# ddrainer/FloodPlanet_Code

Hardware: AMD Instinct MI355X
Metric: training tiles/sec (256x256x8ch UNet) (higher is better)
Workload: dtype bf16; 1 GPU; UNet depth-4 (17.27M params), 8-band 256x256 tiles, batch 16/GPU, fwd+CE(ignore_index=0)+bwd+Adam, train-mode BN; global_batch=16, parallelism=dp1

## Files before the change

floodplanet_code_amd/_lib.py:

```python
from __future__ import annotations

import ctypes as C
import os
from typing import Optional

_HERE = os.path.dirname(os.path.abspath(__file__))
LIB_PATH = os.environ.get("FU_LIB_PATH") or os.path.join(_HERE, "libfloodunet.so")

FU_OK, FU_ERR_INVALID, FU_ERR_HIP, FU_ERR_STATE, FU_ERR_UNSUPPORTED = 0, 1, 2, 3, 4
FU_F32, FU_BF16, FU_F16 = 0, 1, 2
PRECISIONS = {"fp32": FU_F32, "f32": FU_F32, "float32": FU_F32, "bf16": FU_BF16, "bfloat16": FU_BF16,
              "fp16": FU_F16, "f16": FU_F16, "float16": FU_F16, "half": FU_F16}


class FuConfig(C.Structure):
    _fields_ = [
        ("struct_size", C.c_int32),
        ("n_channels", C.c_int32),
        ("n_classes", C.c_int32),
        ("base_channels", C.c_int32),
        ("bilinear", C.c_int32),
        ("max_batch", C.c_int32),
        ("height", C.c_int32),
        ("width", C.c_int32),
# ... 126 lines not shown
    "fu_profile_enable": (_i, [_p, _i]),
    "fu_test_force_general_conv": (None, [_i]),
    "fu_test_force_lockstep_wgrad": (None, [_i]),
    "fu_test_conv_tile_mode": (None, [_i]),
    "fu_test_bnb_separate": (None, [_i]),
    "fu_test_head_store_g": (None, [_i]),
    "fu_test_force_full_taps": (None, [_i]),
    "fu_test_perturb_bnb_sums": (None, [_f]),
    "fu_test_get_buffer": (_i, [_p, _i, _i, C.POINTER(_p), C.POINTER(_i64)]),
    "fu_set_side_stream": (_i, [_p, _i]),
    "fu_backward_join": (_i, [_p, _p]),
    "fu_backward_fence": (_i, [_p, _p, _p]),
    "fu_dp_unique_id": (_i, [_p]),
    "fu_dp_init": (_i, [_p, _p, _i, _i]),
    "fu_dp_broadcast_state": (_i, [_p, _p]),
    "fu_allreduce_begin": (_i, [_p, _i64, _i64, _p]),
    "fu_allreduce_wait": (_i, [_p, _p]),
    "fu_dp_destroy": (_i, [_p]),
    "fu_set_exact_sync": (_i, [_p, SYNC_HOOK, _p, _i, _p, _i64]),
    "fu_exact_sync_bytes": (_i64, [_p]),
    "fu_profile_read": (_i, [_p, _i, C.POINTER(_i64), C.POINTER(C.c_double), C.POINTER(C.c_double),
                             C.POINTER(C.c_char_p)]),
    "fu_elem_size": (_i, [_i]),
    "fu_op_nchw_to_nhwc": (_i, [_i, _p, _p, _i, _i, _i, _i, _i, _p]),
    "fu_op_nhwc_to_nchw": (_i, [_i, _p, _p, _i, _i, _i, _i, _i, _p]),
    "fu_op_conv3x3_fwd": (_i, [_i, _p, _i, _p, _p, _p, _i, _p, _p, _p, _i, _i, _i, _i, _p, _p, _p]),
    "fu_op_conv3x3_dgrad": (_i, [_i, _p, _i, _p, _p, _i, _p, _i, _i, _i, _i, _p]),
    "fu_op_conv3x3_wgrad": (_i, [_i, _p, _i, _p, _p, _p, _i, _p, _i, _p, _i, _i, _i, _p]),
    "fu_op_conv3x3_dgrad_bnsums": (_i, [_i, _p, _i, _p, _p, _i, _p, _p, _p, _p, _p, _p, _p, _i, _i, _i, _p]),
    "fu_op_head_bwd": (_i, [_i, _p, _p, _p, _p, _p, _i, _i, _i64, _p, _p, _p, _p, _p, _p, _p, _p]),
    "fu_op_bn_bwd": (_i, [_i, _p, _p, _i, _i, _i, _i, _p, _p, _p, _p, _p, _p, _p, _p]),
    "fu_op_maxpool2": (_i, [_i, _p, _p, _p, _p, _i, _i, _i, _i, _p]),
    "fu_op_upsample2": (_i, [_i, _p, _p, _p, _p, _i, _i, _i, _i, _i, _i, _p]),
}

_lib: Optional[C.CDLL] = None


def load() -> C.CDLL:
    global _lib
    if _lib is not None:
        return _lib
    if not os.path.exists(LIB_PATH):
        raise RuntimeError(
            f"{LIB_PATH} not found: the HIP extension has not been built. Run "
            "`python -c 'import __graft_entry__ as g; g.build()'` (or `make -C floodplanet_code_amd/csrc`). "
            "There is no CPU / PyTorch fallback for this path.")
    import torch
    lib = C.CDLL(LIB_PATH)
    for name, (res, args) in SIGNATURES.items():
        fn = getattr(lib, name)
        fn.restype = res
        fn.argtypes = args
    _lib = lib
    return lib


def check(status: int) -> None:
    if status != FU_OK:
        msg = load().fu_last_error()
        raise FloodUNetError(status, msg.decode("utf-8", "replace") if msg else "")


def ptr(t) -> Optional[int]:
    return None if t is None else t.data_ptr()
```

floodplanet_code_amd/csrc/fu_api.hip:

```cpp
#include "../../include/floodunet.h"
#include "fu_common.h"
#include <stdlib.h>

#include <math.h>
#include <string.h>

#include <string>
#include <vector>

using namespace fu;

namespace fu {

int conv3x3_num_stat_tiles(Prec p, int B, int H, int W) {
  return p == PREC_F32 ? conv3x3_num_stat_tiles_f32(B, H, W)
                       : (p == PREC_BF16 ? conv3x3_num_stat_tiles_bf16(B, H, W) : conv3x3_num_stat_tiles_f16(B, H, W));
}
int launch_conv3x3(Prec p, const ConvIn& in, const void* wpk, const float* bias, void* dst0, int D0, void* dst1,
                   int D1, float* stats, int* n_stat_tiles, int B, int H, int W, hipStream_t s) {
  if (p == PREC_F32)
    return launch_conv3x3_f32(in, (const float*)wpk, bias, (float*)dst0, D0, (float*)dst1, D1, stats, n_stat_tiles, B,
                              H, W, s);
  if (p == PREC_BF16)
    return launch_conv3x3_bf16(in, (const bf16_t*)wpk, bias, (bf16_t*)dst0, D0, (bf16_t*)dst1, D1, stats, n_stat_tiles,
// ... 162 lines not shown
  const int c = blockIdx.x * blockDim.x + threadIdx.x;
  if (c >= C) return;
  const float invstd = (float)(1.0 / sqrt((double)rv[c] + (double)eps));
  const float sc = gamma[c] * invstd;
  scale[c] = sc;
  fbias[c] = fmaf(sc, bias[c], beta[c] - rm[c] * sc);
  a[c] = 1.f;
  b[c] = 0.f;
}

struct ParamInfo {
  std::string name;
  int ndim;
  int64_t shape[4];
  int64_t off, numel;
};
struct BnInfo {
  std::string name;
  int C;
  int64_t off;
};

struct Conv {
  int cin_real = 0, cin_pad = 0, cout = 0, level = 0;
  int p_w = -1, p_b = -1, p_g = -1, p_beta = -1, bn = -1;
  void* wf = nullptr;
  void* wd = nullptr;
  float *mean = nullptr, *invstd = nullptr, *a = nullptr, *b = nullptr, *coef = nullptr;
  float *fold_scale = nullptr, *fold_bias = nullptr;
  void* y = nullptr;
  void* gy = nullptr;
  const void* pool_g = nullptr;
  int bnb_tiles = 0;
  HeadGrad head;
};

enum BlockKind { BK_INC = 0, BK_DOWN = 1, BK_UP = 2 };

struct Block {
  Conv c[2];
  int kind = BK_INC, level = 0;
  int enc = 0;
  int role = 0;
  int skip = -1;
  void* pooled = nullptr;
  void* g_pooled = nullptr;
  void* up = nullptr;
  void* g_up = nullptr;
  UpTables upt;
  int ct_w = -1, ct_b = -1, ct_cin = 0, ct_cout = 0;
  void* u = nullptr;
  void* g_u = nullptr;
  float* ct_w3 = nullptr;
  float* ct_dw3 = nullptr;
  float* ct_b4 = nullptr;
  void* ct_wf = nullptr;
  void* ct_wd = nullptr;
  int first_param = 0, num_params = 0;
};

struct Fuse {
  int p_w = -1, p_b = -1, C = 0;
  void* cat = nullptr;
  void* gcat = nullptr;
  void* y = nullptr;
  void* gy = nullptr;
// ... 42 lines not shown
struct Dp;
struct fu_ctx {
  fu_config cfg;
  Prec prec;
  size_t esize;
  int Hs[5], Ws[5], ch[5];
  int nE = 1;
  bool fusion = false;
  int nb = 9;
  int enc_ch[FU_MAX_ENCODERS] = {0}, enc_coff[FU_MAX_ENCODERS] = {0}, cin_pad0[FU_MAX_ENCODERS] = {0};
  void* xin[FU_MAX_ENCODERS] = {nullptr};
  std::vector<ParamInfo> params;
  std::vector<BnInfo> bns;
  int64_t total_params = 0, total_bn = 0;
  std::vector<Block> blk;
  Fuse fuse[5];
  int p_outw = -1, p_outb = -1;
  float* P = nullptr;
  float* G = nullptr;
  float* RM = nullptr;
  float* RV = nullptr;
  int64_t* NBT = nullptr;
  bool packed_dirty = true;
  bool packed_eval = false;
  Arena arena;
  std::vector<void*> extra_allocs;
  float* logits = nullptr;
  float* dlogits = nullptr;
  float* dlogits_eff = nullptr;
  float* up_scale = nullptr;
  bool have_up_scale = false;
  float* stats = nullptr;
  float* bnb_part = nullptr;
  int64_t bnb_cap = 0;
  float* db_part = nullptr;
  float* db_part2 = nullptr;
  hipStream_t side = nullptr;
  hipStream_t side_lo = nullptr;
  hipStream_t side_def = nullptr;
  hipEvent_t ev_gy = nullptr, ev_wg[2] = {nullptr, nullptr}, ev_blk = nullptr;
  hipEvent_t ev_fence[2] = {nullptr, nullptr};
  int wg_parity = 0;
  int side_mode = 1;
  bool wg_pending[2] = {false, false};
  double* dscratch = nullptr;
  fu::SyncDesc sync;
  float* slab = nullptr;
  float* ce_part = nullptr;
  float* hb_part = nullptr;
  float* loss_dev = nullptr;
  float* ce_wsum = nullptr;
  float* loss_scale = nullptr;
  int* guard = nullptr;
  unsigned long long* conf_tmp = nullptr;
  int64_t* n_valid = nullptr;
  DeviceTable stitch_table, scene_table, train_table;
  float* adam_m = nullptr;
  float* adam_v = nullptr;
  Profiler prof;
  struct Dp* dp = nullptr;
  std::vector<PackTable> pack_tabs;
  int last_batch = 0;
  int view_n = 0;
  int view_batch = 0;
  unsigned view_codes = 0;
  bool fwd_training = false;
// ... 474 lines not shown
                         f.n_classes, B, f.height, f.width, c->logits, logits_out, s));
  c->last_batch = B;
  c->view_n = n_views;
  c->view_batch = n_views > 0 ? B / n_views : 0;
  c->view_codes = view_codes;
  c->fwd_training = training;
  c->have_loss = false;
  c->have_up_scale = false;
  return 0;
}

static int g_bnb_separate = 0;
static int g_head_store_g = 0;
static float g_test_perturb_bnb = 1.f;
__global__ void k_scale_floats(float* x, int64_t n, float f) {
  for (int64_t i = (int64_t)blockIdx.x * blockDim.x + threadIdx.x; i < n; i += (int64_t)gridDim.x * blockDim.x) x[i] *= f;
}
int perturb_bnb(float* part, int tiles, int C, hipStream_t s) {
  if (g_test_perturb_bnb == 1.f || tiles <= 0) return 0;
  hipLaunchKernelGGL(k_scale_floats, dim3(256), dim3(256), 0, s, part, (int64_t)tiles * C * 2, g_test_perturb_bnb);
  return hipGetLastError() == hipSuccess ? 0 : FU_ERR_HIP;
}

int backward_conv(fu_ctx* c, int i, int j, int B, hipStream_t s) {
  Block& K = c->blk[i];
  Conv& v = K.c[j];
  const int H = c->Hs[v.level], W = c->Ws[v.level];
  const int64_t npix = (int64_t)B * H * W;
  int ndb = 0;
  const bool side = c->side != nullptr && c->side_mode != 0;
  const int par = c->wg_parity;
  float* dbp = (side && par) ? c->db_part2 : c->db_part;
  if (side && c->wg_pending[par]) FU_HIP_CHECK(hipStreamWaitEvent(s, c->ev_wg[par], 0));
  FU_TRY(launch_bn_bwd(c->prec, v.gy, v.y, v.cout, npix, v.a, v.b, v.mean, v.invstd, P(c, v.p_g), G(c, v.p_g),
                       G(c, v.p_beta), c->bnb_part, v.coef, dbp, &ndb, c->dscratch, s, v.pool_g, B, H, W, v.bnb_tiles,
                       v.head.dl ? &v.head : nullptr));
  v.pool_g = nullptr;
  v.bnb_tiles = 0;
  v.head = HeadGrad{};
  ConvIn in = conv_input(c, i, j);
  const double fl = 2.0 * 9 * v.cin_real * v.cout * (double)B * H * W;
  hipStream_t ws = s;
  if (side) {
    FU_HIP_CHECK(hipEventRecord(c->ev_gy, s));
    FU_HIP_CHECK(hipStreamWaitEvent(c->side, c->ev_gy, 0));
    ws = c->side;
  }
  in.opt.prof = prof_arm(c, FU_K_WGRAD, fl);
  FU_TRY(launch_conv3x3_wgrad(c->prec, in, v.gy, v.cout, c->slab, G(c, v.p_w), v.cin_real, dbp, ndb,
                              G(c, v.p_b), B, H, W, ws));
  if (side) {
    FU_HIP_CHECK(hipEventRecord(c->ev_wg[par], c->side));
    c->wg_pending[par] = true;
    c->wg_parity ^= 1;
  }
  ConvIn din{v.gy, v.cout, nullptr, nullptr, nullptr, 0};
  if (!(K.role == 0 && j == 0)) din.opt.prof = prof_arm(c, FU_K_CONV3X3, fl);
  if (j == 1) {
    Conv& v0 = K.c[0];
    const bool separate = g_bnb_separate != 0;
    int tiles = 0;
    BnbFuse f;
    if (c->prec != PREC_F32 && !c->sync.hook && !separate) {
      f.y = v0.y; f.a = v0.a; f.b = v0.b; f.mean = v0.mean; f.invstd = v0.invstd;
      f.part = c->bnb_part; f.max_elems = c->bnb_cap; f.tiles_out = &tiles;
      din.opt.bnb = &f;
    }
    FU_TRY(launch_conv3x3(c->prec, din, v.wd, nullptr, v0.gy, v0.cout, nullptr, 0, nullptr, nullptr, B, H, W, s));
    v0.bnb_tiles = tiles;
    FU_TRY(perturb_bnb(c->bnb_part, tiles, v0.cout, s));
  } else if (K.kind == BK_DOWN) {
    FU_TRY(launch_conv3x3(c->prec, din, v.wd, nullptr, K.g_pooled, v.cin_real, nullptr, 0, nullptr, nullptr, B, H, W,
                          s));
    Conv& pv = c->blk[i - 1].c[1];
    pv.pool_g = K.g_pooled;
  } else if (K.kind == BK_UP) {
    const Feat sk = level_feat(c, K.skip);
    const Feat pv = low_feat(c, i);
    FU_TRY(launch_conv3x3(c->prec, din, v.wd, nullptr, sk.gy, sk.C, K.g_up, v.cin_real - sk.C, nullptr, nullptr,
                          B, H, W, s));
    const int h = c->Hs[K.level + 1], w = c->Ws[K.level + 1];
    if (c->cfg.bilinear) {
      FU_TRY(launch_upsample2_bwd(c->prec, K.g_up, pv.gy, B, h, w, pv.C, H, W, K.upt, s));
    } else {
      FU_TRY(launch_space_to_depth(c->prec, K.g_up, K.g_u, B, h, w, K.ct_cout, H, W, s));
      int ndbp = 0;
      FU_TRY(launch_channel_partial_sums(c->prec, K.g_u, K.ct_cout, (int64_t)B * h * w * 4, c->db_part, &ndbp, s));
      FU_TRY(launch_colsum_partials(c->db_part, ndbp, K.ct_cout, G(c, K.ct_b), s));
      ConvIn lin{pv.y, pv.C, pv.a, pv.b, nullptr, 0, true};
      FU_TRY(launch_conv3x3_wgrad(c->prec, lin, K.g_u, 4 * K.ct_cout, c->slab, K.ct_dw3, K.ct_cin, nullptr, 0, nullptr, B, h,
                                  w, s));
      FU_TRY(launch_convT_grad_from_w3(K.ct_dw3, K.ct_cin, K.ct_cout, G(c, K.ct_w), s));
      ConvIn gin{K.g_u, 4 * K.ct_cout, nullptr, nullptr, nullptr, 0, true};
      FU_TRY(launch_conv3x3(c->prec, gin, K.ct_wd, nullptr, pv.gy, K.ct_cin, nullptr, 0, nullptr, nullptr, B, h, w, s));
    }
  }
  return 0;
}

int num_backward_blocks(const fu_ctx* c) { return 5 + (c->fusion ? 1 : 0) + 5 * c->nE; }
int backward_block_index(const fu_ctx* c, int block) {
  if (block <= 4) return c->nb - block;
  const int k = block - 5 - (c->fusion ? 1 : 0);
  return 5 * c->nE - 1 - k;
}

int backward_block_impl(fu_ctx* c, int block, const float* dlogits_ext, hipStream_t s, bool join) {
  const fu_config& f = c->cfg;
  const int B = c->last_batch;
  if (block == 0) {
    if (dlogits_ext) {
      FU_TRY(launch_dlogits_from_nchw(dlogits_ext, c->dlogits, f.n_classes, B, f.height, f.width, s));
      c->have_up_scale = false;
    } else {
      FU_REQUIRE(c->have_loss, "fu_backward: no dlogits given and no fu_loss_* call since the last forward");
    }
    const float* dl = c->dlogits;
    if (c->prec == PREC_F16 || c->have_up_scale) {
      FU_TRY(launch_loss_grad_eff(c->dlogits, c->dlogits_eff, (int64_t)B * f.height * f.width * f.n_classes,
                                  c->have_up_scale ? c->up_scale : nullptr, c->ce_part,
                                  c->prec == PREC_F16 ? c->loss_scale : nullptr, s,
                                  c->prec == PREC_F16 ? c->guard : nullptr));
      dl = c->dlogits_eff;
    }
    Conv& last = c->blk[c->nb - 1].c[1];
    BnbFuse fz;
    int tiles = 0;
    const bool want = c->prec != PREC_F32 && !c->sync.hook && !g_bnb_separate;
    if (want) {
      fz.y = last.y; fz.a = last.a; fz.b = last.b; fz.mean = last.mean; fz.invstd = last.invstd;
      fz.part = c->bnb_part; fz.max_elems = c->bnb_cap; fz.tiles_out = &tiles;
      fz.skip_g = last.cout % 8 == 0 && 2048 % last.cout == 0 && !g_head_store_g;
    }
    FU_TRY(launch_head_bwd(c->prec, dl, last.y, last.a, last.b, P(c, c->p_outw), f.base_channels, f.n_classes,
                           (int64_t)B * f.height * f.width, last.gy, c->hb_part, G(c, c->p_outw), G(c, c->p_outb), s,
                           want ? &fz : nullptr));
    last.bnb_tiles = tiles;
    FU_REQUIRE(!(want && fz.skip_g) || tiles > 0, "head backward: the fused BatchNorm sums were refused (partials %lld floats)",
               (long long)c->bnb_cap);
    last.head = HeadGrad{};
    if (want && fz.skip_g) { last.head.dl = dl; last.head.w = P(c, c->p_outw); last.head.ncls = f.n_classes; }
    FU_TRY(perturb_bnb(c->bnb_part, tiles, last.cout, s));
    return 0;
// ... 934 lines not shown
  FU_TRY(launch_head_bwd(p, dlogits_nhwc, y, bn_a, bn_b, w, C, ncls, npix, g, (float*)part.p, dw, db, s,
                         want ? &f : nullptr));
  if (want) {
    if (tiles <= 0) {
      set_error("fu_op_head_bwd: the head-backward kernel does not emit the sums in this precision");
      return FU_ERR_UNSUPPORTED;
    }
    FU_TRY(perturb_bnb((float*)bpart.p, tiles, C, s));
    FU_TRY(collapse_partials((const float*)bpart.p, tiles, C, sum_gm, sum_gmx, s));
  }
  FU_HIP_CHECK(hipStreamSynchronize(s));
  return FU_OK;
}

int fu_op_bn_bwd(int precision, void* g, const void* y, int C, int B, int H, int W, const float* bn_a,
                 const float* bn_b, const float* mean, const float* invstd, const void* g_pool, float* dgamma,
                 float* dbeta, fu_stream stream) {
  Prec p; FU_TRY(prec_of(precision, &p));
  FU_REQUIRE(g && y && bn_a && bn_b && mean && invstd && dgamma && dbeta, "fu_op_bn_bwd: null argument");
  hipStream_t s = (hipStream_t)stream;
  const int64_t npix = (int64_t)B * H * W;
  TmpBuf part, coef, dbp, scr;
  FU_TRY(part.get((size_t)bn_bwd_partial_elems(C, npix) * sizeof(float)));
  FU_TRY(coef.get((size_t)C * 2 * sizeof(float)));
  FU_TRY(dbp.get((size_t)bn_bwd_partial_elems(C, npix) * sizeof(float)));
  FU_TRY(scr.get((size_t)reduce_scratch_elems(std::max(C, 64)) * sizeof(double)));
  int ndb = 0;
  FU_TRY(launch_bn_bwd(p, g, y, C, npix, bn_a, bn_b, mean, invstd, nullptr, dgamma, dbeta, (float*)part.p,
                       (float*)coef.p, (float*)dbp.p, &ndb, (double*)scr.p, s, g_pool, B, H, W, 0));
  FU_HIP_CHECK(hipStreamSynchronize(s));
  return FU_OK;
}

int fu_test_get_buffer(fu_ctx* c, int block, int which, void** ptr, int64_t* elems) {
  FU_REQUIRE(c && ptr && elems, "fu_test_get_buffer: null argument");
  FU_REQUIRE(block >= 0 && block < c->nb, "fu_test_get_buffer: block %d outside 0..%d", block, c->nb - 1);
  const Block& K = c->blk[block];
  const int B = c->cfg.max_batch;
  auto act = [&](int level, int C) { return (int64_t)B * c->Hs[level] * c->Ws[level] * C; };
  switch (which) {
    case 0: *ptr = K.c[0].y; *elems = act(K.c[0].level, K.c[0].cout); break;
    case 1: *ptr = K.c[0].gy; *elems = act(K.c[0].level, K.c[0].cout); break;
    case 2: *ptr = K.c[1].y; *elems = act(K.c[1].level, K.c[1].cout); break;
    case 3: *ptr = K.c[1].gy; *elems = act(K.c[1].level, K.c[1].cout); break;
    case 4: *ptr = K.g_pooled; *elems = K.kind == BK_DOWN ? act(K.level, K.c[0].cin_real) : 0; break;
    case 5: *ptr = K.g_up; *elems = K.kind == BK_UP ? act(K.level, K.c[0].cin_real - c->ch[K.skip]) : 0; break;
    default: set_error("fu_test_get_buffer: which must be 0..5"); return FU_ERR_INVALID;
  }
  return FU_OK;
}

}

extern "C" void fu_test_bnb_separate(int on) { g_bnb_separate = on ? 1 : 0; }
extern "C" void fu_test_head_store_g(int on) { g_head_store_g = on ? 1 : 0; }
extern "C" void fu_test_perturb_bnb_sums(float factor) { g_test_perturb_bnb = factor; }
```

floodplanet_code_amd/csrc/fu_common.h:

```cpp
#pragma once
#include <hip/hip_runtime.h>
#include <stdint.h>
#include <stdio.h>
#include <string>

struct fu_stitch_entry;
struct fu_scene_crop;
struct fu_scene_train_entry;

namespace fu {

typedef unsigned short bf16_t;
struct f16_t { unsigned short v; };

enum Prec { PREC_F32 = 0, PREC_BF16 = 1, PREC_F16 = 2 };

template <typename F> auto dispatch_prec(Prec p, F&& f) {
  if (p == PREC_F32) return f(float{});
  if (p == PREC_BF16) return f(bf16_t{});
  return f(f16_t{});
}

void set_error(const char* fmt, ...);
const char* get_error();
// ... 300 lines not shown
                        int src_channels = 0, int src_channel_offset = 0);
int launch_nhwc_to_nchw(Prec p, const void* src, float* dst, int B, int C, int H, int W, int c_pad, hipStream_t s);
struct SrcList { const float* p[8]; int c[8]; int coff[9]; int n; };
int launch_gather_nchw_to_nhwc(Prec p, const SrcList& S, void* dst, int B, int C, int H, int W, int c_pad, int ch_off,
                               hipStream_t s);
int launch_gather_views_nchw_to_nhwc(Prec p, const SrcList& S, void* dst, int B, int n_views, unsigned codes, int C, int H,
                                     int W, int c_pad, int ch_off, hipStream_t s);

int launch_bn_finalize(const float* partials, int nTiles, int C, int64_t count, const float* conv_bias,
                       const float* gamma, const float* beta, float eps, float momentum, float* mean, float* invstd,
                       float* a, float* b, float* running_mean, float* running_var, int64_t* nbt, double* dscratch,
                       hipStream_t s);
static inline int64_t reduce_scratch_elems(int C) { return (int64_t)32 * C * 2; }
int64_t bn_bwd_partial_elems(int C, int64_t npix);
int launch_bn_bwd(Prec p, void* g, const void* y, int C, int64_t npix, const float* a, const float* b,
                  const float* mean, const float* invstd, const float* gamma, float* dgamma, float* dbeta,
                  float* partials, float* coef, float* db_partials, int* n_db_partials, double* dscratch,
                  hipStream_t s, const void* g_pool = nullptr, int B = 0, int H = 0, int W = 0, int ext_partials = 0,
                  const HeadGrad* head = nullptr);

int launch_maxpool2(Prec p, const void* src, const float* a, const float* b, void* dst, int B, int H, int W, int C,
                    hipStream_t s);
struct UpTables {
  const int* y_i0; const int* y_i1; const float* y_w1;
  const int* x_i0; const int* x_i1; const float* x_w1;
  const int* yb_o; const float* yb_w;
  const int* xb_o; const float* xb_w;
  float scale_y, scale_x;
};
static constexpr int UP_BWD_MAX = 6;
int launch_upsample2(Prec p, const void* src, const float* a, const float* b, void* dst, int B, int H, int W, int C,
                     int outH, int outW, const UpTables& t, hipStream_t s);
int launch_upsample2_bwd(Prec p, const void* g_dst, void* g_src, int B, int H, int W, int C, int outH, int outW,
                         const UpTables& t, hipStream_t s);

int launch_depth_to_space(Prec p, const void* y4, void* up, int B, int h, int w, int C, int outH, int outW, hipStream_t s);
int launch_space_to_depth(Prec p, const void* gup, void* g4, int B, int h, int w, int C, int outH, int outW, hipStream_t s);
int launch_colsum_partials(const float* partials, int n, int C, float* out, hipStream_t s);
int launch_channel_partial_sums(Prec p, const void* g, int C, int64_t npix, float* partials, int* n_partials,
                                hipStream_t s);
int launch_convT_to_w3(const float* w, const float* b, int Cin, int Cout, float* w3, float* bias4, hipStream_t s);
int launch_convT_grad_from_w3(const float* dw3, int Cin, int Cout, float* dw, hipStream_t s);
int launch_copy_channels(Prec p, const void* src, int srcC, int src_off, const float* a, const float* b, void* dst,
                         int dstC, int dst_off, int C, int64_t npix, hipStream_t s);
int launch_center_to_w3(const float* w, int64_t n, float* w3, hipStream_t s);
int launch_center_from_w3(const float* dw3, int64_t n, float* dw, hipStream_t s);

int launch_head_fwd(Prec p, const void* y, const float* a, const float* b, const float* w, const float* bias, int C,
                    int ncls, int B, int H, int W, float* logits_nhwc, float* logits_nchw, hipStream_t s);
static constexpr int HEAD_MAX_CLS = 8;
int launch_ce_loss(const float* logits_nhwc, const int64_t* target, int ncls, int ignore_index, int64_t npix,
                   float* partials, float* loss_out, int64_t* n_valid_dev, int64_t* confusion_accum,
                   int64_t* n_valid_out, unsigned long long* conf_tmp , hipStream_t s);
int launch_ce_grad(const float* logits_nhwc, const int64_t* target, int ncls, int ignore_index, int64_t npix,
                   const int64_t* n_valid_dev, float* dlogits_nhwc, hipStream_t s);
int launch_ce_weighted_loss(const float* logits_nhwc, const int64_t* target, int ncls, int ignore_index, int64_t npix,
                            const float* class_weight, float c_nll, float c_smooth, float* partials ,
                            float* loss_out, int64_t* n_valid_dev, float* weight_sum_dev, int64_t* confusion_accum,
                            int64_t* n_valid_out, float* weight_sum_out, unsigned long long* conf_tmp, hipStream_t s);
int launch_ce_weighted_grad(const float* logits_nhwc, const int64_t* target, int ncls, int ignore_index, int64_t npix,
                            const float* class_weight, float c_nll, float c_smooth, const float* weight_sum_dev,
                            float* dlogits_nhwc, hipStream_t s);
int launch_bce_dice(const float* logits_nhwc, const int64_t* target, int ncls, int ignore_index, int64_t npix,
                    float dice_w, float* partials, float* coef, float* loss_out, int64_t* n_valid_dev,
                    float* dlogits_nhwc, hipStream_t s);
int launch_dlogits_from_nchw(const float* dlogits_nchw, float* dlogits_nhwc, int ncls, int B, int H, int W,
                             hipStream_t s);
// ... 47 lines not shown
```

floodplanet_code_amd/csrc/fu_elementwise.hip:

```cpp
#include "fu_common.h"

#include <stdarg.h>

namespace fu {

thread_local const SyncDesc* g_sync = nullptr;
thread_local const float* g_grad_unscale = nullptr;

int sync_sum_over_ranks(void* payload, int64_t n_elems, bool is_double, hipStream_t s) {
  const SyncDesc* d = g_sync;
  if (!d || !d->hook || d->world <= 1) return 0;
  const size_t bytes = (size_t)n_elems * (is_double ? 8 : 4);
  FU_REQUIRE((int64_t)bytes <= d->xbytes, "exact sync: exchange buffer too small (%zu > %lld bytes)", bytes,
             (long long)d->xbytes);
  FU_HIP_CHECK(hipMemcpyAsync(d->xbuf, payload, bytes, hipMemcpyDeviceToDevice, s));
  if (d->hook(d->user, n_elems, is_double ? 1 : 0) != 0) {
    set_error("exact sync: the all-reduce hook failed");
    return 3;
  }
  FU_HIP_CHECK(hipMemcpyAsync(payload, d->xbuf, bytes, hipMemcpyDeviceToDevice, s));
  return 0;
}

static thread_local char g_err[1024] = "";
// ... 826 lines not shown
  float z00[R][V], z01[R][V], z10[R][V], z11[R][V], wy1[R];
  bool in[R];
#pragma unroll
  for (int r = 0; r < R; ++r) {
    const int uy = oy0 + r - py0;
    in[r] = in_x && uy >= 0 && uy < 2 * H && oy0 + r < outH;
    const float sy = t.scale_y * (float)uy;
    const int y0 = in[r] ? (int)sy : 0;
    const int y1 = y0 + (y0 < H - 1 ? 1 : 0);
    wy1[r] = fminf(fmaxf(sy - (float)y0, 0.f), 1.f);
    VecIO<T>::load(base + ((size_t)y0 * W + x0) * C, z00[r]);
    VecIO<T>::load(base + ((size_t)y0 * W + x1) * C, z01[r]);
    VecIO<T>::load(base + ((size_t)y1 * W + x0) * C, z10[r]);
    VecIO<T>::load(base + ((size_t)y1 * W + x1) * C, z11[r]);
  }
#pragma unroll
  for (int r = 0; r < R; ++r) {
    if (oy0 + r >= outH) break;
    float o[V];
    const float wy0 = 1.f - wy1[r];
#pragma unroll
    for (int j = 0; j < V; ++j) {
      float p00 = z00[r][j], p01 = z01[r][j], p10 = z10[r][j], p11 = z11[r][j];
      if (bn) {
        p00 = bn_act(av[j], p00, bv[j]); p01 = bn_act(av[j], p01, bv[j]);
        p10 = bn_act(av[j], p10, bv[j]); p11 = bn_act(av[j], p11, bv[j]);
      }
      o[j] = in[r] ? wy0 * (wx0 * p00 + wx1 * p01) + wy1[r] * (wx0 * p10 + wx1 * p11) : 0.f;
    }
    VecIO<T>::store(dst + ((size_t)(bb * outH + oy0 + r) * outW + ox) * C + cv * V, o);
  }
}

template <typename T>
__global__ __launch_bounds__(256) void k_upsample2_bwd(const T* __restrict__ gdst, T* __restrict__ gsrc, int H, int W,
                                                       int C, int outH, int outW, int py0, int px0, UpTables t, int CV,
                                                       unsigned rcpCV) {
  constexpr int V = VecIO<T>::V;
  const int item = blockIdx.x * 256 + threadIdx.x;
  if (item >= W * CV) return;
  const int ix = fast_div(item, CV, rcpCV), cv = item - ix * CV;
  const int iy = blockIdx.y, bb = blockIdx.z;
  float acc[V];
#pragma unroll
  for (int j = 0; j < V; ++j) acc[j] = 0.f;
  const T* base = gdst + (size_t)bb * outH * outW * C + cv * V;
  int xo[UP_BWD_MAX];
  float xw[UP_BWD_MAX];
#pragma unroll
  for (int jx = 0; jx < UP_BWD_MAX; ++jx) { xo[jx] = t.xb_o[ix * UP_BWD_MAX + jx]; xw[jx] = t.xb_w[ix * UP_BWD_MAX + jx]; }
  for (int jy = 0; jy < UP_BWD_MAX; ++jy) {
    const int oy = t.yb_o[iy * UP_BWD_MAX + jy];
    if (oy < 0) break;
    const float wy = t.yb_w[iy * UP_BWD_MAX + jy];
    const T* rowp = base + (size_t)(oy + py0) * outW * C;
#pragma unroll
    for (int jx = 0; jx < UP_BWD_MAX; ++jx) {
      if (__builtin_amdgcn_ballot_w64(xo[jx] >= 0) == 0) break;
      if (xo[jx] >= 0) {
        const float w = wy * xw[jx];
        float gv[V];
        VecIO<T>::load(rowp + (size_t)(xo[jx] + px0) * C, gv);
#pragma unroll
        for (int j = 0; j < V; ++j) acc[j] += w * gv[j];
      }
    }
  }
  VecIO<T>::store(gsrc + ((size_t)(bb * H + iy) * W + ix) * C + cv * V, acc);
}

int launch_upsample2(Prec p, const void* src, const float* a, const float* b, void* dst, int B, int H, int W, int C,
                     int outH, int outW, const UpTables& t, hipStream_t s) {
  FU_REQUIRE(outH >= 2 * H && outW >= 2 * W, "upsample: target smaller than 2x source");
  const int py0 = (outH - 2 * H) / 2, px0 = (outW - 2 * W) / 2;
  return dispatch_prec(p, [&](auto tag) {
    using T = decltype(tag);
    dim3 g; int CV; unsigned rcp;
    FU_REQUIRE(row_grid<T>(C, outW, outH, B, &g, &CV, &rcp), "upsample: unsupported shape (C=%d H=%d B=%d)", C, outH, B);
    if ((int64_t)g.x * ceil_div(outH, 4) * B >= 2048) {
      g.y = ceil_div(outH, 4);
      hipLaunchKernelGGL((k_upsample2<T, 4>), g, dim3(256), 0, s, (const T*)src, a, b, (T*)dst, H, W, C, outH, outW, py0, px0,
                         t, CV, rcp);
    } else {
      hipLaunchKernelGGL((k_upsample2<T, 1>), g, dim3(256), 0, s, (const T*)src, a, b, (T*)dst, H, W, C, outH, outW, py0, px0,
                         t, CV, rcp);
    }
    FU_LAUNCH_CHECK();
    return 0;
  });
}

int launch_upsample2_bwd(Prec p, const void* g_dst, void* g_src, int B, int H, int W, int C, int outH, int outW,
                         const UpTables& t, hipStream_t s) {
  const int py0 = (outH - 2 * H) / 2, px0 = (outW - 2 * W) / 2;
  return dispatch_prec(p, [&](auto tag) {
    using T = decltype(tag);
    dim3 g; int CV; unsigned rcp;
    FU_REQUIRE(row_grid<T>(C, W, H, B, &g, &CV, &rcp), "upsample_bwd: unsupported shape (C=%d H=%d B=%d)", C, H, B);
    hipLaunchKernelGGL(k_upsample2_bwd<T>, g, dim3(256), 0, s, (const T*)g_dst, (T*)g_src, H, W, C, outH, outW, py0, px0, t,
                       CV, rcp);
    FU_LAUNCH_CHECK();
    return 0;
  });
}

template <typename T>
__global__ void k_depth_to_space(const T* __restrict__ y4, T* __restrict__ up, int h, int w, int C, int outH, int outW,
                                 int py0, int px0, int64_t total) {
  const int CV = C >> 2;
  for (int64_t idx = (int64_t)blockIdx.x * blockDim.x + threadIdx.x; idx < total;
       idx += (int64_t)gridDim.x * blockDim.x) {
    const int cv = (int)(idx % CV);
    int64_t r = idx / CV;
    const int ox = (int)(r % outW); r /= outW;
    const int oy = (int)(r % outH);
    const int64_t bb = r / outH;
    float o[4] = {0, 0, 0, 0};
    const int uy = oy - py0, ux = ox - px0;
    if (uy >= 0 && uy < 2 * h && ux >= 0 && ux < 2 * w) {
      const int ph = (uy & 1) * 2 + (ux & 1);
      ElemIO<T>::load4(y4 + (((bb * h + (uy >> 1)) * w + (ux >> 1)) * 4 + ph) * (int64_t)C + cv * 4, o);
    }
    ElemIO<T>::store4(up + idx * 4, o);
  }
}
template <typename T>
__global__ void k_space_to_depth(const T* __restrict__ gup, T* __restrict__ g4, int h, int w, int C, int outH, int outW,
                                 int py0, int px0, int64_t total) {
  const int CV = C >> 2;
  for (int64_t idx = (int64_t)blockIdx.x * blockDim.x + threadIdx.x; idx < total;
       idx += (int64_t)gridDim.x * blockDim.x) {
    const int cv = (int)(idx % CV);
    int64_t r = idx / CV;
// ... 1097 lines not shown
```

include/floodunet.h:

```cpp
#ifndef FLOODUNET_H_
#define FLOODUNET_H_

#include <stddef.h>
#include <stdint.h>

#ifdef __cplusplus
extern "C" {
#endif

#define FU_ABI_VERSION 5
#define FU_MAX_ENCODERS 6

typedef struct fu_ctx fu_ctx;
typedef void* fu_stream;

enum fu_status {
  FU_OK = 0,
  FU_ERR_INVALID = 1,
  FU_ERR_HIP = 2,
  FU_ERR_STATE = 3,
  FU_ERR_UNSUPPORTED = 4
};

enum fu_precision {
// ... 169 lines not shown
  FU_K_NUM = 2
};
int fu_profile_enable(fu_ctx* ctx, int enable);
int fu_profile_read(fu_ctx* ctx, int kernel_class, int64_t* launches, double* total_ms, double* total_flops,
                    const char** kernel_name);

void fu_test_force_general_conv(int on);
void fu_test_force_lockstep_wgrad(int on);
void fu_test_conv_tile_mode(int mode);
void fu_test_bnb_separate(int on);
void fu_test_head_store_g(int on);
void fu_test_force_full_taps(int on);

void fu_test_perturb_bnb_sums(float factor);
int fu_test_get_buffer(fu_ctx* ctx, int block, int which, void** ptr, int64_t* elems);

int fu_elem_size(int precision);
int fu_op_nchw_to_nhwc(int precision, const float* src, void* dst, int B, int C, int H, int W, int c_pad,
                       fu_stream stream);
int fu_op_nhwc_to_nchw(int precision, const void* src, float* dst, int B, int C, int H, int W, int c_pad,
                       fu_stream stream);
int fu_op_conv3x3_fwd(int precision, const void* src0, int C0, const float* bn_a0, const float* bn_b0,
                      const void* src1, int C1, const float* w_oihw, const float* bias, void* y, int Cout, int B,
                      int H, int W, float* stats_sum, float* stats_sqsum, fu_stream stream);
int fu_op_conv3x3_dgrad(int precision, const void* dy, int Cout, const float* w_oihw, void* dx0, int C0, void* dx1,
                        int C1, int B, int H, int W, fu_stream stream);
int fu_op_conv3x3_wgrad(int precision, const void* src0, int C0, const float* bn_a0, const float* bn_b0,
                        const void* src1, int C1, const void* dy, int Cout, float* dw_oihw, int B, int H, int W,
                        fu_stream stream);
int fu_op_maxpool2(int precision, const void* src, const float* bn_a, const float* bn_b, void* dst, int B, int H,
                   int W, int C, fu_stream stream);
int fu_op_upsample2(int precision, const void* src, const float* bn_a, const float* bn_b, void* dst, int B, int H,
                    int W, int C, int outH, int outW, fu_stream stream);

int fu_op_conv3x3_dgrad_bnsums(int precision, const void* dy, int Cout, const float* w_oihw, void* dx, int C0,
                               const void* y, const float* bn_a, const float* bn_b, const float* mean,
                               const float* invstd, float* sum_gm, float* sum_gmx, int B, int H, int W,
                               fu_stream stream);
int fu_op_head_bwd(int precision, const float* dlogits_nhwc, const void* y, const float* bn_a, const float* bn_b,
                   const float* w, int C, int ncls, int64_t npix, void* g, float* dw, float* db, const float* mean,
                   const float* invstd, float* sum_gm, float* sum_gmx, fu_stream stream);
int fu_op_bn_bwd(int precision, void* g, const void* y, int C, int B, int H, int W, const float* bn_a,
                 const float* bn_b, const float* mean, const float* invstd, const void* g_pool, float* dgamma,
                 float* dbeta, fu_stream stream);

#ifdef __cplusplus
}
#endif
#endif
```

Measured before the change: 3059 tiles/s.

## Fuse BatchNorm backward partial sums into bilinear upsample backward kernel

Rewrites the bilinear upsample backward kernel as a persistent per-block loop over pixels, with batched 4x4 tap loads and a general fallback path. In 16-bit precisions it also computes the per-channel BN backward reductions (sum of masked grad and grad times normalized x) for the lower-resolution conv output while the gradient is still in registers. The BN backward for that layer then reuses those partials instead of running a separate reduction pass over the data. Ownership checks keep the carried partials from being consumed by the wrong layer. A standalone op entry point is added for testing.

```diff
diff --git a/floodplanet_code_amd/_lib.py b/floodplanet_code_amd/_lib.py
--- a/floodplanet_code_amd/_lib.py
+++ b/floodplanet_code_amd/_lib.py
@@ -182,6 +182,7 @@
     "fu_op_bn_bwd": (_i, [_i, _p, _p, _i, _i, _i, _i, _p, _p, _p, _p, _p, _p, _p, _p]),
     "fu_op_maxpool2": (_i, [_i, _p, _p, _p, _p, _i, _i, _i, _i, _p]),
     "fu_op_upsample2": (_i, [_i, _p, _p, _p, _p, _i, _i, _i, _i, _i, _i, _p]),
+    "fu_op_upsample2_bwd": (_i, [_i, _p, _p, _i, _i, _i, _i, _i, _i, _p, _p, _p, _p, _p, _p, C.POINTER(C.c_int), _p]),
 }
 
 _lib: Optional[C.CDLL] = None
diff --git a/floodplanet_code_amd/csrc/fu_api.hip b/floodplanet_code_amd/csrc/fu_api.hip
--- a/floodplanet_code_amd/csrc/fu_api.hip
+++ b/floodplanet_code_amd/csrc/fu_api.hip
@@ -218,6 +218,7 @@
   void* gy = nullptr;
   const void* pool_g = nullptr;
   int bnb_tiles = 0;
+  bool bnb_from_up = false;
   HeadGrad head;
 };
 
@@ -326,6 +327,7 @@
   bool have_up_scale = false;
   float* stats = nullptr;
   float* bnb_part = nullptr;
+  const void* bnb_owner = nullptr;
   int64_t bnb_cap = 0;
   float* db_part = nullptr;
   float* db_part2 = nullptr;
@@ -866,11 +868,15 @@
   const int par = c->wg_parity;
   float* dbp = (side && par) ? c->db_part2 : c->db_part;
   if (side && c->wg_pending[par]) FU_HIP_CHECK(hipStreamWaitEvent(s, c->ev_wg[par], 0));
+  FU_REQUIRE(c->bnb_owner == nullptr || c->bnb_owner == &v, "backward: carried BatchNorm sums reached another layer's backward first");
+  if (v.bnb_from_up && g_bnb_separate) v.bnb_tiles = 0;
   FU_TRY(launch_bn_bwd(c->prec, v.gy, v.y, v.cout, npix, v.a, v.b, v.mean, v.invstd, P(c, v.p_g), G(c, v.p_g),
                        G(c, v.p_beta), c->bnb_part, v.coef, dbp, &ndb, c->dscratch, s, v.pool_g, B, H, W, v.bnb_tiles,
                        v.head.dl ? &v.head : nullptr));
   v.pool_g = nullptr;
   v.bnb_tiles = 0;
+  v.bnb_from_up = false;
+  c->bnb_owner = nullptr;
   v.head = HeadGrad{};
   ConvIn in = conv_input(c, i, j);
   const double fl = 2.0 * 9 * v.cin_real * v.cout * (double)B * H * W;
@@ -915,7 +921,24 @@
                           B, H, W, s));
     const int h = c->Hs[K.level + 1], w = c->Ws[K.level + 1];
     if (c->cfg.bilinear) {
-      FU_TRY(launch_upsample2_bwd(c->prec, K.g_up, pv.gy, B, h, w, pv.C, H, W, K.upt, s));
+      const bool low_is_conv = !(c->fusion && i == 5 * c->nE);
+      int tiles = 0;
+      BnbFuse f;
+      if (low_is_conv && c->prec != PREC_F32 && !c->sync.hook && !g_bnb_separate) {
+        Conv& lv = c->blk[i - 1].c[1];
+        f.y = lv.y; f.a = lv.a; f.b = lv.b; f.mean = lv.mean; f.invstd = lv.invstd;
+        f.part = c->bnb_part; f.max_elems = c->bnb_cap; f.tiles_out = &tiles;
+      }
+      FU_TRY(launch_upsample2_bwd(c->prec, K.g_up, pv.gy, B, h, w, pv.C, H, W, K.upt, s, f.tiles_out ? &f : nullptr));
+      if (tiles > 0) {
+        Conv& lv = c->blk[i - 1].c[1];
+        FU_REQUIRE(j == 0 && c->bnb_owner == nullptr && lv.pool_g == nullptr,
+                   "backward: the BatchNorm sums of the resize backward would not reach their consumer first");
+        lv.bnb_tiles = tiles;
+        lv.bnb_from_up = true;
+        c->bnb_owner = &lv;
+        FU_TRY(perturb_bnb(c->bnb_part, tiles, lv.cout, s));
+      }
     } else {
       FU_TRY(launch_space_to_depth(c->prec, K.g_up, K.g_u, B, h, w, K.ct_cout, H, W, s));
       int ndbp = 0;
@@ -943,6 +966,9 @@
   const fu_config& f = c->cfg;
   const int B = c->last_batch;
   if (block == 0) {
+    c->bnb_owner = nullptr;
+    for (Block& K : c->blk)
+      for (Conv& v : K.c) { v.bnb_tiles = 0; v.bnb_from_up = false; }
     if (dlogits_ext) {
       FU_TRY(launch_dlogits_from_nchw(dlogits_ext, c->dlogits, f.n_classes, B, f.height, f.width, s));
       c->have_up_scale = false;
@@ -1943,6 +1969,41 @@
   return FU_OK;
 }
 
+int fu_op_upsample2_bwd(int precision, const void* g_dst, void* g_src, int B, int H, int W, int C, int outH, int outW,
+                        const void* y, const float* bn_a, const float* bn_b, const float* mean, const float* invstd,
+                        float* sums_out, int* tiles_out, fu_stream stream) {
+  Prec p; FU_TRY(prec_of(precision, &p));
+  FU_REQUIRE(g_dst && g_src, "fu_op_upsample2_bwd: null argument");
+  const bool want = y || bn_a || bn_b || mean || invstd || sums_out || tiles_out;
+  FU_REQUIRE(!want || (y && bn_a && bn_b && mean && invstd && sums_out && tiles_out),
+             "fu_op_upsample2_bwd: the fused sums need y, a, b, mean, invstd, sums_out and tiles_out together");
+  FU_REQUIRE(!want || p != PREC_F32, "fu_op_upsample2_bwd: fused sums in the 16-bit precisions only (fp32 keeps the separate reduce pass)");
+  hipStream_t s = (hipStream_t)stream;
+  fu_ctx tmp;
+  UpTables t;
+  TmpBuf part;
+  int st = build_up_tables(&tmp, H, W, &t);
+  int tiles = 0;
+  if (st == 0 && want) {
+    const int64_t cap = (int64_t)std::max(*tiles_out, 0) * C * 2;
+    st = part.get((size_t)std::max<int64_t>(cap, 1) * sizeof(float));
+    if (st == 0) {
+      BnbFuse f;
+      f.y = y; f.a = bn_a; f.b = bn_b; f.mean = mean; f.invstd = invstd;
+      f.part = (float*)part.p; f.max_elems = cap; f.tiles_out = &tiles;
+      st = launch_upsample2_bwd(p, g_dst, g_src, B, H, W, C, outH, outW, t, s, &f);
+      if (st == 0 && tiles > 0) st = perturb_bnb((float*)part.p, tiles, C, s);
+      if (st == 0 && tiles > 0) st = collapse_partials((const float*)part.p, tiles, C, sums_out, sums_out + C, s);
+      *tiles_out = tiles;
+    }
+  } else if (st == 0) {
+    st = launch_upsample2_bwd(p, g_dst, g_src, B, H, W, C, outH, outW, t, s);
+  }
+  (void)hipStreamSynchronize(s);
+  for (void* q : tmp.extra_allocs) (void)hipFree(q);
+  return st;
+}
+
 int fu_test_get_buffer(fu_ctx* c, int block, int which, void** ptr, int64_t* elems) {
   FU_REQUIRE(c && ptr && elems, "fu_test_get_buffer: null argument");
   FU_REQUIRE(block >= 0 && block < c->nb, "fu_test_get_buffer: block %d outside 0..%d", block, c->nb - 1);
diff --git a/floodplanet_code_amd/csrc/fu_common.h b/floodplanet_code_amd/csrc/fu_common.h
--- a/floodplanet_code_amd/csrc/fu_common.h
+++ b/floodplanet_code_amd/csrc/fu_common.h
@@ -356,7 +356,7 @@
 int launch_upsample2(Prec p, const void* src, const float* a, const float* b, void* dst, int B, int H, int W, int C,
                      int outH, int outW, const UpTables& t, hipStream_t s);
 int launch_upsample2_bwd(Prec p, const void* g_dst, void* g_src, int B, int H, int W, int C, int outH, int outW,
-                         const UpTables& t, hipStream_t s);
+                         const UpTables& t, hipStream_t s, const BnbFuse* fuse = nullptr);
 
 int launch_depth_to_space(Prec p, const void* y4, void* up, int B, int h, int w, int C, int outH, int outW, hipStream_t s);
 int launch_space_to_depth(Prec p, const void* gup, void* g4, int B, int h, int w, int C, int outH, int outW, hipStream_t s);
diff --git a/floodplanet_code_amd/csrc/fu_elementwise.hip b/floodplanet_code_amd/csrc/fu_elementwise.hip
--- a/floodplanet_code_amd/csrc/fu_elementwise.hip
+++ b/floodplanet_code_amd/csrc/fu_elementwise.hip
@@ -882,41 +882,165 @@
   }
 }
 
+struct UpBwdGeom {
+  int H, W, C, outW, py0, px0, CV;
+  int npix, per_wg;
+  unsigned img_stride;
+  unsigned rcpW, rcpH;
+};
+
 template <typename T>
-__global__ __launch_bounds__(256) void k_upsample2_bwd(const T* __restrict__ gdst, T* __restrict__ gsrc, int H, int W,
-                                                       int C, int outH, int outW, int py0, int px0, UpTables t, int CV,
-                                                       unsigned rcpCV) {
+__device__ __forceinline__ void up_bwd_unpack(const uint4& r, float (&v)[VecIO<T>::V]) {
+  if constexpr (sizeof(T) == 4) {
+    v[0] = __uint_as_float(r.x); v[1] = __uint_as_float(r.y); v[2] = __uint_as_float(r.z); v[3] = __uint_as_float(r.w);
+  } else if constexpr (std::is_same<T, bf16_t>::value) {
+    v[0] = __uint_as_float(r.x << 16); v[1] = __uint_as_float(r.x & 0xffff0000u);
+    v[2] = __uint_as_float(r.y << 16); v[3] = __uint_as_float(r.y & 0xffff0000u);
+    v[4] = __uint_as_float(r.z << 16); v[5] = __uint_as_float(r.z & 0xffff0000u);
+    v[6] = __uint_as_float(r.w << 16); v[7] = __uint_as_float(r.w & 0xffff0000u);
+  } else {
+    unpack_h2(r.x, v[0], v[1]); unpack_h2(r.y, v[2], v[3]); unpack_h2(r.z, v[4], v[5]); unpack_h2(r.w, v[6], v[7]);
+  }
+}
+
+__device__ __forceinline__ int up_bwd_off(const UpBwdGeom& G, int oy, int ox) {
+  return ((max(oy, 0) + G.py0) * G.outW + max(ox, 0) + G.px0) * G.C;
+}
+
+template <typename T>
+__device__ __forceinline__ void up_bwd_taps4(const T* __restrict__ img, const UpBwdGeom& G, const int (&yo)[UP_BWD_MAX],
+                                             const float (&yw)[UP_BWD_MAX], const int (&xo)[UP_BWD_MAX],
+                                             const float (&xw)[UP_BWD_MAX], float (&acc)[VecIO<T>::V]) {
   constexpr int V = VecIO<T>::V;
-  const int item = blockIdx.x * 256 + threadIdx.x;
-  if (item >= W * CV) return;
-  const int ix = fast_div(item, CV, rcpCV), cv = item - ix * CV;
-  const int iy = blockIdx.y, bb = blockIdx.z;
-  float acc[V];
-#pragma unroll
-  for (int j = 0; j < V; ++j) acc[j] = 0.f;
-  const T* base = gdst + (size_t)bb * outH * outW * C + cv * V;
-  int xo[UP_BWD_MAX];
-  float xw[UP_BWD_MAX];
-#pragma unroll
-  for (int jx = 0; jx < UP_BWD_MAX; ++jx) { xo[jx] = t.xb_o[ix * UP_BWD_MAX + jx]; xw[jx] = t.xb_w[ix * UP_BWD_MAX + jx]; }
+  constexpr int NT = 4;
+  uint4 raw[NT * NT];
+#pragma unroll
+  for (int jy = 0; jy < NT; ++jy)
+#pragma unroll
+    for (int jx = 0; jx < NT; ++jx) raw[jy * NT + jx] = *reinterpret_cast<const uint4*>(img + up_bwd_off(G, yo[jy], xo[jx]));
+#pragma unroll
+  for (int jy = 0; jy < NT; ++jy)
+#pragma unroll
+    for (int jx = 0; jx < NT; ++jx) {
+      const bool ok = yo[jy] >= 0 && xo[jx] >= 0;
+      const float w = yw[jy] * xw[jx];
+      float gv[V];
+      up_bwd_unpack<T>(raw[jy * NT + jx], gv);
+#pragma unroll
+      for (int j = 0; j < V; ++j) acc[j] = ok ? acc[j] + w * gv[j] : acc[j];
+    }
+}
+
+template <typename T>
+__device__ __forceinline__ void up_bwd_taps_any(const T* __restrict__ img, const UpBwdGeom& G, const UpTables& t, int iy,
+                                                const int (&xo)[UP_BWD_MAX], const float (&xw)[UP_BWD_MAX],
+                                                float (&acc)[VecIO<T>::V]) {
+  constexpr int V = VecIO<T>::V;
+#pragma unroll 1
   for (int jy = 0; jy < UP_BWD_MAX; ++jy) {
     const int oy = t.yb_o[iy * UP_BWD_MAX + jy];
-    if (oy < 0) break;
     const float wy = t.yb_w[iy * UP_BWD_MAX + jy];
-    const T* rowp = base + (size_t)(oy + py0) * outW * C;
+    if (__builtin_amdgcn_ballot_w64(oy >= 0) == 0) break;
+    uint4 raw[UP_BWD_MAX];
+#pragma unroll
+    for (int jx = 0; jx < UP_BWD_MAX; ++jx) raw[jx] = *reinterpret_cast<const uint4*>(img + up_bwd_off(G, oy, xo[jx]));
 #pragma unroll
     for (int jx = 0; jx < UP_BWD_MAX; ++jx) {
-      if (__builtin_amdgcn_ballot_w64(xo[jx] >= 0) == 0) break;
-      if (xo[jx] >= 0) {
-        const float w = wy * xw[jx];
-        float gv[V];
-        VecIO<T>::load(rowp + (size_t)(xo[jx] + px0) * C, gv);
-#pragma unroll
-        for (int j = 0; j < V; ++j) acc[j] += w * gv[j];
+      const bool ok = oy >= 0 && xo[jx] >= 0;
+      const float w = wy * xw[jx];
+      float gv[V];
+      up_bwd_unpack<T>(raw[jx], gv);
+#pragma unroll
+      for (int j = 0; j < V; ++j) acc[j] = ok ? acc[j] + w * gv[j] : acc[j];
+    }
+  }
+}
+
+template <typename T, bool BNB>
+__global__ __launch_bounds__(BNB_THREADS) void k_upsample2_bwd(const T* __restrict__ gdst, T* __restrict__ gsrc, UpBwdGeom G,
+                                                               UpTables t, const T* __restrict__ y,
+                                                               const float* __restrict__ a, const float* __restrict__ b,
+                                                               const float* __restrict__ mean,
+                                                               const float* __restrict__ invstd,
+                                                               float* __restrict__ partials) {
+  extern __shared__ float sm[];
+  constexpr int V = VecIO<T>::V;
+  const int rows = BNB_THREADS / G.CV;
+  const int cv = threadIdx.x % G.CV, row = threadIdx.x / G.CV;
+  const int bid = xcd_remap(blockIdx.x, gridDim.x);
+  float s1[V], s2[V], av[V], bv[V], mv[V], iv[V];
+  if constexpr (BNB) {
+#pragma unroll
+    for (int j = 0; j < V; ++j) s1[j] = s2[j] = 0.f;
+  }
+  if (row < rows) {
+    if constexpr (BNB) {
+#pragma unroll
+      for (int q = 0; q < V; q += 4) {
+        float t4[4];
+        ElemIO<float>::load4(a + cv * V + q, t4);
+        for (int j = 0; j < 4; ++j) av[q + j] = t4[j];
+        ElemIO<float>::load4(b + cv * V + q, t4);
+        for (int j = 0; j < 4; ++j) bv[q + j] = t4[j];
+        ElemIO<float>::load4(mean + cv * V + q, t4);
+        for (int j = 0; j < 4; ++j) mv[q + j] = t4[j];
+        ElemIO<float>::load4(invstd + cv * V + q, t4);
+        for (int j = 0; j < 4; ++j) iv[q + j] = t4[j];
       }
     }
-  }
-  VecIO<T>::store(gsrc + ((size_t)(bb * H + iy) * W + ix) * C + cv * V, acc);
+    for (int k = 0; k < G.per_wg; ++k) {
+      const int p = (bid * G.per_wg + k) * rows + row;
+      if (p >= G.npix) break;
+      const int q = fast_div(p, G.W, G.rcpW), ix = p - q * G.W;
+      const int bb = fast_div(q, G.H, G.rcpH), iy = q - bb * G.H;
+      int yo[UP_BWD_MAX], xo[UP_BWD_MAX];
+      float yw[UP_BWD_MAX], xw[UP_BWD_MAX];
+#pragma unroll
+      for (int j = 0; j < UP_BWD_MAX; ++j) {
+        yo[j] = t.yb_o[iy * UP_BWD_MAX + j]; yw[j] = t.yb_w[iy * UP_BWD_MAX + j];
+        xo[j] = t.xb_o[ix * UP_BWD_MAX + j]; xw[j] = t.xb_w[ix * UP_BWD_MAX + j];
+      }
+      float yv[V];
+      if constexpr (BNB) VecIO<T>::load(y + (size_t)p * G.C + cv * V, yv);
+      float acc[V];
+#pragma unroll
+      for (int j = 0; j < V; ++j) acc[j] = 0.f;
+      const T* img = gdst + (size_t)bb * G.img_stride + cv * V;
+      if (__builtin_amdgcn_ballot_w64(yo[4] >= 0 || xo[4] >= 0) == 0)
+        up_bwd_taps4<T>(img, G, yo, yw, xo, xw, acc);
+      else
+        up_bwd_taps_any<T>(img, G, t, iy, xo, xw, acc);
+      VecIO<T>::store(gsrc + (size_t)p * G.C + cv * V, acc);
+      if constexpr (BNB) {
+#pragma unroll
+        for (int j = 0; j < V; ++j) {
+          const float z = bn_act_pre(av[j], yv[j], bv[j]);
+          const float gm = z > 0.f ? acc[j] : 0.f;
+          s1[j] += gm;
+          s2[j] += gm * ((yv[j] - mv[j]) * iv[j]);
+        }
+      }
+    }
+    if constexpr (BNB) {
+#pragma unroll
+      for (int j = 0; j < V; ++j) {
+        sm[((row * G.C) + cv * V + j) * 2 + 0] = s1[j];
+        sm[((row * G.C) + cv * V + j) * 2 + 1] = s2[j];
+      }
+    }
+  }
+  if constexpr (BNB) {
+    __syncthreads();
+    for (int c = threadIdx.x; c < G.C; c += BNB_THREADS) {
+      float t1 = 0.f, t2 = 0.f;
+      for (int r = 0; r < rows; ++r) {
+        t1 += sm[(r * G.C + c) * 2 + 0];
+        t2 += sm[(r * G.C + c) * 2 + 1];
+      }
+      partials[((int64_t)blockIdx.x * G.C + c) * 2 + 0] = t1;
+      partials[((int64_t)blockIdx.x * G.C + c) * 2 + 1] = t2;
+    }
+  }
 }
 
 int launch_upsample2(Prec p, const void* src, const float* a, const float* b, void* dst, int B, int H, int W, int C,
@@ -941,14 +1065,35 @@
 }
 
 int launch_upsample2_bwd(Prec p, const void* g_dst, void* g_src, int B, int H, int W, int C, int outH, int outW,
-                         const UpTables& t, hipStream_t s) {
-  const int py0 = (outH - 2 * H) / 2, px0 = (outW - 2 * W) / 2;
+                         const UpTables& t, hipStream_t s, const BnbFuse* fuse) {
+  FU_REQUIRE(outH >= 2 * H && outW >= 2 * W, "upsample_bwd: target smaller than 2x source");
+  const int64_t npix = (int64_t)B * H * W;
   return dispatch_prec(p, [&](auto tag) {
     using T = decltype(tag);
-    dim3 g; int CV; unsigned rcp;
-    FU_REQUIRE(row_grid<T>(C, W, H, B, &g, &CV, &rcp), "upsample_bwd: unsupported shape (C=%d H=%d B=%d)", C, H, B);
-    hipLaunchKernelGGL(k_upsample2_bwd<T>, g, dim3(256), 0, s, (const T*)g_dst, (T*)g_src, H, W, C, outH, outW, py0, px0, t,
-                       CV, rcp);
+    constexpr int V = 16 / (int)sizeof(T);
+    FU_REQUIRE(C % V == 0 && C / V <= BNB_THREADS && C % 4 == 0 && C <= 1024, "upsample_bwd: unsupported channel count %d", C);
+    FU_REQUIRE((int64_t)outH * outW * C < ((int64_t)1 << 31) && npix < ((int64_t)1 << 30) && npix * W < ((int64_t)1 << 32) &&
+                   (int64_t)B * H * H < ((int64_t)1 << 32),
+               "upsample_bwd: tensor too large for 32-bit indexing (B=%d H=%d W=%d C=%d)", B, H, W, C);
+    UpBwdGeom G;
+    G.H = H; G.W = W; G.C = C; G.outW = outW; G.py0 = (outH - 2 * H) / 2; G.px0 = (outW - 2 * W) / 2; G.CV = C / V;
+    G.npix = (int)npix; G.img_stride = (unsigned)((int64_t)outH * outW * C);
+    G.rcpW = host_rcp(W); G.rcpH = host_rcp(H);
+    const int nb = bn_bwd_blocks(C, npix);
+    const int rows = BNB_THREADS / G.CV;
+    G.per_wg = (int)ceil_div64(npix, (int64_t)nb * rows);
+    bool sums = false;
+    if constexpr (sizeof(T) == 2) sums = fuse && fuse->part && fuse->tiles_out && (int64_t)nb * C * 2 <= fuse->max_elems;
+    if (fuse && fuse->tiles_out) *fuse->tiles_out = 0;
+    if (sums) {
+      const size_t sh = (size_t)rows * C * 2 * sizeof(float);
+      hipLaunchKernelGGL((k_upsample2_bwd<T, true>), dim3(nb), dim3(BNB_THREADS), sh, s, (const T*)g_dst, (T*)g_src, G, t,
+                         (const T*)fuse->y, fuse->a, fuse->b, fuse->mean, fuse->invstd, fuse->part);
+      *fuse->tiles_out = nb;
+    } else {
+      hipLaunchKernelGGL((k_upsample2_bwd<T, false>), dim3(nb), dim3(BNB_THREADS), 0, s, (const T*)g_dst, (T*)g_src, G, t,
+                         (const T*)nullptr, nullptr, nullptr, nullptr, nullptr, nullptr);
+    }
     FU_LAUNCH_CHECK();
     return 0;
   });
diff --git a/include/floodunet.h b/include/floodunet.h
--- a/include/floodunet.h
+++ b/include/floodunet.h
@@ -225,6 +225,9 @@
                    int W, int C, fu_stream stream);
 int fu_op_upsample2(int precision, const void* src, const float* bn_a, const float* bn_b, void* dst, int B, int H,
                     int W, int C, int outH, int outW, fu_stream stream);
+int fu_op_upsample2_bwd(int precision, const void* g_dst, void* g_src, int B, int H, int W, int C, int outH, int outW,
+                        const void* y, const float* bn_a, const float* bn_b, const float* mean, const float* invstd,
+                        float* sums_out, int* tiles_out, fu_stream stream);
 
 int fu_op_conv3x3_dgrad_bnsums(int precision, const void* dy, int Cout, const float* w_oihw, void* dx, int C0,
                                const void* y, const float* bn_a, const float* bn_b, const float* mean,
```

New measurement: 3057 tiles/s. About the same (-0.1%).
